# jakub-zarzycki2022/gym-PBN-stac

Measured on AMD Instinct MI355X. Metric: env-steps/sec (whole node), Bittner-200, batch=1M; achieved HBM GB/s, higher is better.
Workload: dtype u64; 1 GPU; Bittner-200 async node update (R1 Graph.step), step mode: one update per env per launch, state resident in device memory; network=bittner199, n_nodes=199, state_words=4, batch_per_gpu=1048576, global_batch=1048576, parallelism=dp1 (env shards, no collective), rng=philox4x32-10

## Files before the change

gym-pbn-stac_amd/csrc/pbn_abi.cpp:

```cpp
#include "pbn_host.hpp"

#include <cstdlib>

const void* DevCache::on(int device, const void* host, size_t bytes) {
    std::lock_guard<std::mutex> g(mu);
    auto it = dev.find(device);
    if (it != dev.end()) return it->second;
    void* p = nullptr;
    if (hipMalloc(&p, bytes) != hipSuccess) return nullptr;
    if (hipMemcpy(p, host, bytes, hipMemcpyHostToDevice) != hipSuccess) {
        (void)hipFree(p);
        return nullptr;
    }
    dev[device] = p;
    return p;
}

void DevCache::release() {
    for (auto& kv : dev) {
        (void)hipSetDevice(kv.first);
        (void)hipFree(kv.second);
    }
    dev.clear();
}
// ... 5 lines not shown
    if (const char* v = getenv("PBNSIM_STEP_BLOCK")) k.step_block = atoi(v) == 256 ? 256 : 1024;
    k.env_no_gen = getenv("PBNSIM_ENV_NO_GEN") != nullptr;
    if (const char* v = getenv("PBNSIM_ENV_GROUP")) k.env_group = std::max(1, atoi(v));
    if (const char* v = getenv("PBNSIM_ENV_BPC")) k.env_bpc = std::max(1, atoi(v));
    if (const char* v = getenv("PBNSIM_ENV_CHUNK")) k.env_chunk = atoi(v);
    if (const char* v = getenv("PBNSIM_ENV_GRID")) k.env_grid_cap = std::max(1, atoi(v));
    if (const char* v = getenv("PBNSIM_ENV_TAIL")) k.env_tail = std::max(0, std::min(64, atoi(v)));
    if (const char* v = getenv("PBNSIM_ENV_LANES")) k.env_lane_limit = std::max(0, std::min(64, atoi(v)));
    if (const char* v = getenv("PBNSIM_ENV_STEAL")) k.env_steal = atoi(v) != 0;
    if (const char* v = getenv("PBNSIM_ENV_KERNEL_IMAGE")) k.env_kernel_image = atoi(v) != 0;
    if (const char* v = getenv("PBNSIM_ENV_HELPERS")) k.env_helpers = std::max(0, std::min(3, atoi(v)));
    if (const char* v = getenv("PBNSIM_ENV_GRID_STEAL")) k.env_grid_steal = atoi(v) != 0 ? 1 : 0;
#ifdef PBN_MEASURE_KNOBS
    if (const char* v = getenv("PBNSIM_ENV_POOL_CU_IDLE")) k.env_pool_cu_idle = atoi(v) != 0 ? 1 : 0;
    if (const char* v = getenv("PBNSIM_ENV_GRID_SLOTS")) k.env_grid_slots = std::max(1, std::min((int)GPOOL_CAP, atoi(v)));
#endif
    if (const char* v = getenv("PBNSIM_SSD_WAVE")) k.ssd_wave = atoi(v) ? 1 : 0;
    if (const char* v = getenv("PBNSIM_SSD_SERIAL")) k.ssd_serial = atoi(v) != 0;
    if (const char* v = getenv("PBNSIM_SSD_SHARED")) {
        const int w = atoi(v);
        k.ssd_shared = w == 0 ? 0 : (w == 4 || w == 8) ? w : 1;
    }
    if (const char* v = getenv("PBNSIM_STEP_GRAPH")) k.step_graph = atoi(v) != 0 ? 1 : 0;
    if (const char* v = getenv("PBNSIM_MT_LANES")) k.mt_lane_walk = atoi(v) != 0;
    if (const char* v = getenv("PBNSIM_ROLL_GROUP")) k.roll_group = std::max(0, atoi(v));
    return k;
}

static bool roll_group_ok(const pbn_net* net) { return net->kind == PBN_KIND_PREDICTOR_MIX && net->N <= 256; }

static int roll_group_size(const pbn_batch* b, const pbn_net* net) {
    if (!roll_group_ok(net)) return 1;
    const uint64_t lanes = (uint64_t)b->n_cu * 512u;
    for (int g = 8; g >= 2; g /= 2)
        if (b->B * (uint64_t)g <= lanes) return g;
    return 1;
}

static int check_state_words(const pbn_batch* b, const uint64_t* w) {
    const int r = b->N & 63;
    if (!r) return 0;
    const uint64_t bad = ~(((uint64_t)1 << r) - 1);
    for (uint64_t e = 0; e < b->B; e++)
        if (w[e * b->W + b->W - 1] & bad) return fail(PBN_E_RANGE, "env %llu has bits set beyond node %d",
                                                       (unsigned long long)e, b->N - 1);
    return 0;
}

int h2d(pbn_batch* b, void* dst, const void* src, size_t bytes) {
    if (bytes <= PinBuf::CAP && b->pin.ready()) {
        HIP_TRY(hipStreamSynchronize(b->stream));
        memcpy(b->pin.p, src, bytes);
        HIP_TRY(hipMemcpyAsync(dst, b->pin.p, bytes, hipMemcpyHostToDevice, b->stream));
    } else {
        HIP_TRY(hipMemcpyAsync(dst, src, bytes, hipMemcpyHostToDevice, b->stream));
    }
    return 0;
}

// ... 106 lines not shown
    if (n_envs < 1) return fail(PBN_E_INVALID, "n_envs must be >= 1");
    if (env_id_base + n_envs > ((uint64_t)1 << 56)) return fail(PBN_E_RANGE, "global env ids must stay below 2^56");
    if (int rc = open_device(device)) return rc;
    pbn_batch* b = new pbn_batch;
    b->net = net;
    b->device = device;
    b->W = net->W;
    b->N = net->N;
    b->B = n_envs;
    b->env_base = env_id_base;
    b->seed = seed;
    b->knob = read_knobs();
    hipDeviceProp_t prop;
    int rc = 0;
    auto bail = [&](int code) {
        pbn_batch_destroy(b);
        return code;
    };
    if (hipGetDeviceProperties(&prop, device) != hipSuccess) return bail(fail(PBN_E_HIP, "hipGetDeviceProperties"));
    b->n_cu = prop.multiProcessorCount;
    if (b->knob.step_block)
        b->step_block = b->knob.step_block;
    else
        b->step_block = n_envs >= (uint64_t)b->n_cu * 1024u * (uint64_t)b->knob.envs_per_thread ? 1024 : 256;
    b->sg.off = b->knob.step_graph >= 0 ? b->knob.step_graph == 0 : n_envs * (uint64_t)b->W >= STEP_GRAPH_MAX_WORDS;
    b->roll_group = roll_group_size(b, net);
    if (b->knob.roll_group >= 0) {
        const int g = b->knob.roll_group;
        b->roll_group = (g == 2 || g == 4 || g == 8) && roll_group_ok(net) ? g : 1;
    }
    if (hipStreamCreateWithFlags(&b->stream, hipStreamNonBlocking) != hipSuccess)
        return bail(fail(PBN_E_HIP, "hipStreamCreate"));
    b->own_stream = b->stream;
    size_t sb = 8 * (size_t)b->W * n_envs;
    if (hipMalloc(&b->d_state, sb) != hipSuccess) return bail(fail(PBN_E_NOMEM, "state alloc (%zu B)", sb));
    if (hipMalloc(&b->d_nsteps, 8 * n_envs) != hipSuccess) return bail(fail(PBN_E_NOMEM, "n_steps alloc"));
    if (hipMalloc(&b->d_error, 8) != hipSuccess) return bail(fail(PBN_E_NOMEM, "error flag alloc"));
    if (hipMemsetAsync(b->d_error, 0, 8, b->stream) != hipSuccess || hipMemsetAsync(b->d_state, 0, sb, b->stream) != hipSuccess ||
        hipMemsetAsync(b->d_nsteps, 0, 8 * n_envs, b->stream) != hipSuccess)
        return bail(fail(PBN_E_HIP, "hipMemset"));
    b->d_image = net->image_on(device);
    if (!b->d_image) return bail(fail(PBN_E_NOMEM, "network image upload failed"));
    if ((rc = max_blocks_step(b->W, net->kind, net->L.bytes, BLOCK, &b->bpc_base)))
        return bail(fail(PBN_E_HIP, "occupancy query: %s", hipGetErrorString((hipError_t)rc)));
    if ((rc = max_blocks_step(b->W, net->kind, net->L.plane_off, b->step_block, &b->bpc_step)))
        return bail(fail(PBN_E_HIP, "occupancy query: %s", hipGetErrorString((hipError_t)rc)));
    if ((rc = max_blocks_step(b->W, net->kind, net->L.plane_off, BLOCK, &b->bpc_roll, 1, b->roll_group)))
        return bail(fail(PBN_E_HIP, "occupancy query: %s", hipGetErrorString((hipError_t)rc)));
    if (hipStreamSynchronize(b->stream) != hipSuccess) return bail(fail(PBN_E_HIP, "stream sync"));
    *out = b;
    return 0;
}
void pbn_batch_destroy(pbn_batch* b) {
    if (!b) return;
    (void)hipSetDevice(b->device);
    if (b->stream) (void)hipStreamSynchronize(b->stream);
    for (auto& pr : b->tm.ev_pool) {
        (void)hipEventDestroy(pr.first);
        (void)hipEventDestroy(pr.second);
    }
    if (b->d_state) (void)hipFree(b->d_state);
    if (b->d_nsteps) (void)hipFree(b->d_nsteps);
    if (b->d_error) (void)hipFree(b->d_error);
    for (DevBuf* d : {&b->s_act, &b->s_obs, &b->s_rew, &b->s_flags, &b->s_nup, &b->s_replay_i, &b->s_replay_k,
                      &b->s_off, &b->s_mask, &b->mt.py, &b->mt.np, &b->mt.pos_py, &b->mt.pos_np, &b->mt.seeds,
                      &b->r6.counter, &b->r6.steal, &b->r6.gpool, &b->aux.ssd_hist, &b->aux.ssd_tab, &b->aux.sync_tab, &b->sg.ubase, &b->s_flip_err})
        d->release();
    for (hipGraphExec_t& g : b->sg.graph)
        if (g) (void)hipGraphExecDestroy(g);
    for (hipGraphExec_t& g : b->sg.exact_graph)
        if (g) (void)hipGraphExecDestroy(g);
    b->pin.release();
    if (b->own_stream) {
        (void)hipStreamSynchronize(b->stream);
        (void)hipStreamDestroy(b->own_stream);
    }
    delete b;
}

int pbn_batch_set_stream(pbn_batch* b, int own, void* stream) {
    CHECK_NN(b, "batch");
    hipStream_t s = own ? b->own_stream : (hipStream_t)stream;
    if (s == b->stream) return 0;
    SET_DEV(b);
    HIP_TRY(hipStreamSynchronize(b->stream));
    b->stream = s;
    return 0;
}

int pbn_batch_get_info(const pbn_batch* b, pbn_batch_info* info) {
    CHECK_NN(b, "batch");
    CHECK_NN(info, "info");
    info->n_nodes = b->N;
    info->n_words = b->W;
    info->kind = b->net->kind;
    info->device = b->device;
    info->n_envs = b->B;
    info->env_id_base = b->env_base;
    info->seed = b->seed;
    info->update_count = b->update_count;
    info->env_call_count = b->r6.calls;
    info->reset_count = b->reset_count;
    info->mt_ready = b->mt.ready;
    const EnvPlan& p = b->r6.last;
    info->env_lanes = p.grp;
    info->roll_lanes = b->roll_group;
    info->env_grid = p.grid;
    info->env_kernel = p.kernel;
    info->env_lane_limit = (int)p.lane_limit;
    info->env_handoff = p.handoff ? 1 : 0;
    info->env_chunk = (p.mode == ENV_MODE_COOP || p.mode == ENV_MODE_TAIL) ? (int)p.chunk : 0;
    return 0;
}

int pbn_sync(pbn_batch* b) {
    CHECK_NN(b, "batch");
    SET_DEV(b);
    HIP_TRY(hipStreamSynchronize(b->stream));
    if (b->r6.fault_check) {
        b->r6.fault_check = false;
        int32_t f = 0;
        HIP_TRY(hipMemcpy(&f, b->d_error + 1, 4, hipMemcpyDeviceToHost));
        if (f) {
            HIP_TRY(hipMemset(b->d_error + 1, 0, 4));
            return fail(PBN_E_HIP, "k_env grid pool: a wait timed out in a device-path launch (an env's outputs "
                                   "were not written)");
        }
    }
    return 0;
}

int pbn_set_state(pbn_batch* b, const uint64_t* words) {
    CHECK_NN(b, "batch");
    CHECK_NN(words, "words");
// ... 190 lines not shown
```

gym-pbn-stac_amd/csrc/pbn_abi_sim.cpp:

```cpp
#include "pbn_host.hpp"

static int step_launch(pbn_batch* b, uint32_t T, uint64_t update_base, int replay, const void* d_i, const void* d_k,
                       const uint64_t* ubase_dev = nullptr, bool timed = true) {
    StepArgs a{};
    a.ubase_dev = ubase_dev;
    a.state = b->d_state;
    a.img = b->d_image;
    a.L = b->net->L;
    a.B = b->B;
    a.env_base = b->env_base;
    a.seed = b->seed;
    a.update_base = update_base;
    a.T = T;
    a.replay_node = (const uint32_t*)d_i;
    a.replay_k53 = (const uint64_t*)d_k;
    hipEvent_t stop = nullptr;
    if (timed)
        if (int rc = b->ev_begin(&stop)) return rc;
    int store = (T == 1 && !replay) ? b->knob.store_mode : STORE_FULL;
    const bool rollout = T > 1 && !replay;
    a.grp = rollout ? b->roll_group : 1;
    const uint64_t K = rollout ? 1u : (uint64_t)b->knob.envs_per_thread;
    const uint64_t lanes = rollout ? b->B * (uint64_t)a.grp : (b->B + K - 1) / K;
    const int sb = (replay || rollout) ? BLOCK : b->step_block;
    const int grid = replay    ? b->grid_for(lanes, b->bpc_base)
                     : rollout ? b->grid_for(lanes, b->bpc_roll, sb)
                               : b->grid_for(lanes, b->bpc_step, sb);
    int e = launch_step(b->W, a, store, replay, sb, grid, b->stream);
    if (e) return fail(PBN_E_HIP, "k_step launch: %s", hipGetErrorString((hipError_t)e));
    return timed ? b->ev_end(stop) : 0;
}

static bool step_graph_ready(pbn_batch* b) {
    if (b->sg.built) return true;
    if (b->sg.broken || b->sg.off || !b->stream) return false;
    if (b->sg.ubase.ensure(64)) return false;
    bool ok = true;
    for (int j = 0; ok && j < STEP_GRAPH_SIZES; ++j) {
        const uint32_t K = STEP_GRAPH_K >> j;
        hipGraph_t g = nullptr;
        ok = hipStreamBeginCapture(b->stream, hipStreamCaptureModeThreadLocal) == hipSuccess;
        bool launched = ok;
        for (uint32_t k = 0; launched && k < K; ++k)
            launched = step_launch(b, 1, k, 0, nullptr, nullptr, (const uint64_t*)b->sg.ubase.p, false) == 0;
        if (launched) launched = launch_bump((uint64_t*)b->sg.ubase.p, K, b->stream) == 0;
        if (ok) ok = hipStreamEndCapture(b->stream, &g) == hipSuccess && launched && g;
        if (ok) ok = hipGraphInstantiate(&b->sg.graph[j], g, nullptr, nullptr, 0) == hipSuccess;
        if (g) (void)hipGraphDestroy(g);
    }
    if (!ok) {
        for (hipGraphExec_t& g : b->sg.graph) {
            if (g) (void)hipGraphExecDestroy(g);
            g = nullptr;
        }
        b->sg.broken = true;
        (void)hipGetLastError();
        g_err.clear();
        return false;
    }
    b->sg.built = true;
    return true;
}

static int exact_graph_build(pbn_batch* b, uint32_t n) {
    if (n < 2 || n > STEP_GRAPH_K || b->sg.broken || b->sg.off || b->sg.exact_broken || !b->stream)
        return -1;
    if (b->sg.ubase.ensure(64)) return -1;
    hipGraph_t g = nullptr;
    hipGraphExec_t x = nullptr;
    bool ok = hipStreamBeginCapture(b->stream, hipStreamCaptureModeThreadLocal) == hipSuccess;
    bool launched = ok;
    for (uint32_t k = 0; launched && k < n; ++k)
        launched = step_launch(b, 1, k, 0, nullptr, nullptr, (const uint64_t*)b->sg.ubase.p, false) == 0;
    if (ok) ok = hipStreamEndCapture(b->stream, &g) == hipSuccess && launched && g;
    if (ok) ok = hipGraphInstantiate(&x, g, nullptr, nullptr, 0) == hipSuccess;
    if (ok) ok = hipGraphUpload(x, b->stream) == hipSuccess;
    if (g) (void)hipGraphDestroy(g);
    if (!ok) {
        if (x) (void)hipGraphExecDestroy(x);
        b->sg.exact_broken = true;
        (void)hipGetLastError();
        g_err.clear();
        return -1;
    }
    int slot = 0;
    for (int j = 1; j < pbn_batch::StepGraphs::EXACT_GRAPHS; ++j)
        if (b->sg.exact_used[j] < b->sg.exact_used[slot]) slot = j;
    if (b->sg.exact_graph[slot]) {
        if (hipStreamSynchronize(b->stream) != hipSuccess) {
            (void)hipGraphExecDestroy(x);
            (void)fail(PBN_E_HIP, "stream sync before graph eviction failed");
            return -1;
        }
        (void)hipGraphExecDestroy(b->sg.exact_graph[slot]);
    }
    b->sg.exact_graph[slot] = x;
    b->sg.exact_n[slot] = n;
    b->sg.exact_used[slot] = ++b->sg.exact_clock;
    return slot;
}

static int exact_graph_find(pbn_batch* b, uint32_t n) {
    for (int j = 0; j < pbn_batch::StepGraphs::EXACT_GRAPHS; ++j)
        if (b->sg.exact_graph[j] && b->sg.exact_n[j] == n) return j;
    return -1;
}

static bool stream_capturing(pbn_batch* b) {
    hipStreamCaptureStatus cap = hipStreamCaptureStatusNone;
    if (b->stream && hipStreamIsCapturing(b->stream, &cap) != hipSuccess) return true;
    return cap != hipStreamCaptureStatusNone;
}

static int upload_update_count(pbn_batch* b) {
    uint32_t* c = (uint32_t*)b->sg.ubase.p;
    HIP_TRY(hipMemsetD32Async((hipDeviceptr_t)c, (int)(uint32_t)b->update_count, 1, b->stream));
    HIP_TRY(hipMemsetD32Async((hipDeviceptr_t)(c + 1), (int)(uint32_t)(b->update_count >> 32), 1, b->stream));
    return 0;
}

static int check_replay_nodes(const pbn_batch* b, const char* what, const uint32_t* node_idx, const uint64_t* k53,
                              uint64_t n) {
    const uint32_t lo = (uint32_t)b->net->kind == PBN_KIND_PROB_TABLE ? 1u : 0u;
    for (uint64_t q = 0; q < n; q++) {
        if (node_idx[q] >= (uint32_t)b->N || node_idx[q] < lo)
            return fail(PBN_E_RANGE, "%s node index %u outside [%u, %d)", what, node_idx[q], lo, b->N);
        if (k53 && k53[q] >> 53) return fail(PBN_E_RANGE, "replay k53 must be < 2^53");
    }
    return 0;
}

extern "C" {

int pbn_step_prepare(pbn_batch* b, uint32_t n_updates) {
    CHECK_NN(b, "batch");
    if (n_updates > PBN_STEP_PREPARE_MAX)
        return fail(PBN_E_INVALID, "n_updates=%u above PBN_STEP_PREPARE_MAX", n_updates);
    SET_DEV(b);
    if (n_updates < 2 || b->sg.off || stream_capturing(b)) return 0;
    if (n_updates > STEP_GRAPH_K) (void)step_graph_ready(b);
    else if (exact_graph_find(b, n_updates) < 0) (void)exact_graph_build(b, n_updates);
    return 0;
}

int pbn_step(pbn_batch* b, uint32_t n_updates) {
    CHECK_NN(b, "batch");
    SET_DEV(b);
    uint32_t t = 0;
    const bool cap = stream_capturing(b);
    const uint32_t smallest = STEP_GRAPH_K >> (STEP_GRAPH_SIZES - 1);
    int exact = -1;
    if (!cap && b->tm.mode != 1 && n_updates >= 2 && !b->sg.off) {
        exact = exact_graph_find(b, n_updates);
        if (exact < 0 && n_updates == b->sg.last_n && n_updates <= STEP_GRAPH_K)
            exact = exact_graph_build(b, n_updates);
    }
    b->sg.last_n = n_updates;
    if (exact >= 0) {
        if (int rc = upload_update_count(b)) return rc;
        hipEvent_t stop;
        if (int rc = b->ev_begin(&stop)) return rc;
        if (b->tm.mode == 2) b->tm.region_launches += n_updates - 1;
        HIP_TRY(hipGraphLaunch(b->sg.exact_graph[exact], b->stream));
        if (int rc = b->ev_end(stop)) return rc;
        b->sg.exact_used[exact] = ++b->sg.exact_clock;
        b->update_count += n_updates;
        return 0;
    }
    if (n_updates >= smallest && b->tm.mode != 1 && !cap && step_graph_ready(b)) {
        if (int rc = upload_update_count(b)) return rc;
        for (int j = 0; j < STEP_GRAPH_SIZES; ++j) {
            const uint32_t K = STEP_GRAPH_K >> j;
            while (n_updates - t >= K && (j == 0 || n_updates - t < 2 * K)) {
                hipEvent_t stop;
                if (int rc = b->ev_begin(&stop)) return rc;
                if (b->tm.mode == 2) b->tm.region_launches += K - 1;
                HIP_TRY(hipGraphLaunch(b->sg.graph[j], b->stream));
                if (int rc = b->ev_end(stop)) return rc;
                b->update_count += K;
                t += K;
            }
        }
    }
    for (; t < n_updates; t++) {
        if (int rc = step_launch(b, 1, b->update_count, 0, nullptr, nullptr)) return rc;
        b->update_count++;
    }
    return 0;
}

int pbn_rollout(pbn_batch* b, uint32_t n_updates) {
    CHECK_NN(b, "batch");
    if (!n_updates) return 0;
    SET_DEV(b);
    if (int rc = step_launch(b, n_updates, b->update_count, 0, nullptr, nullptr)) return rc;
    b->update_count += n_updates;
    return 0;
}

int pbn_step_replay(pbn_batch* b, const uint32_t* node_idx, const uint64_t* k53, uint32_t n_updates) {
    CHECK_NN(b, "batch");
    if (!n_updates) return 0;
    CHECK_NN(node_idx, "node_idx");
    CHECK_NN(k53, "k53");
    const uint64_t n = (uint64_t)n_updates * b->B;
    if (int rc = check_replay_nodes(b, "replay", node_idx, k53, n)) return rc;
    SET_DEV(b);
    if (int rc = b->s_replay_i.ensure(4 * n)) return rc;
    if (int rc = b->s_replay_k.ensure(8 * n)) return rc;
    HIP_TRY(hipMemcpyAsync(b->s_replay_i.p, node_idx, 4 * n, hipMemcpyHostToDevice, b->stream));
    HIP_TRY(hipMemcpyAsync(b->s_replay_k.p, k53, 8 * n, hipMemcpyHostToDevice, b->stream));
    if (int rc = step_launch(b, n_updates, 0, 1, b->s_replay_i.p, b->s_replay_k.p)) return rc;
    HIP_TRY(hipStreamSynchronize(b->stream));
    return 0;
}

int pbn_step_forced(pbn_batch* b, const uint32_t* node_idx, uint32_t n_updates) {
    CHECK_NN(b, "batch");
    if (!n_updates) return 0;
    CHECK_NN(node_idx, "node_idx");
    const uint64_t n = (uint64_t)n_updates * b->B;
    if (int rc = check_replay_nodes(b, "forced", node_idx, nullptr, n)) return rc;
    SET_DEV(b);
    if (int rc = b->s_replay_i.ensure(4 * n)) return rc;
    HIP_TRY(hipMemcpyAsync(b->s_replay_i.p, node_idx, 4 * n, hipMemcpyHostToDevice, b->stream));
    if (int rc = step_launch(b, n_updates, b->update_count, 1, b->s_replay_i.p, nullptr)) return rc;
    b->update_count += n_updates;
    HIP_TRY(hipStreamSynchronize(b->stream));
    return 0;
}

static MTArgs mt_args(pbn_batch* b) {
    MTArgs a{};
    a.state = b->d_state;
    a.img = b->d_image;
    a.L = b->net->L;
    a.B = b->B;
    a.n_nodes = b->N;
    a.mt_py = (uint32_t*)b->mt.py.p;
    a.mt_np = (uint32_t*)b->mt.np.p;
    a.pos_py = (uint32_t*)b->mt.pos_py.p;
    a.pos_np = (uint32_t*)b->mt.pos_np.p;
    a.lane_walk = b->knob.mt_lane_walk ? 1 : 0;
    return a;
}

int pbn_mt_seed(pbn_batch* b, const uint64_t* seeds, int init_state) {
    CHECK_NN(b, "batch");
    CHECK_NN(seeds, "seeds");
// ... 135 lines not shown
```

gym-pbn-stac_amd/csrc/pbn_host.hpp:

```cpp
#pragma once
#include <algorithm>
#include <cstdint>
#include <cstring>
#include <map>
#include <mutex>
#include <string>
#include <vector>

#ifndef PBN_HOST_NO_HIP
#include <hip/hip_runtime_api.h>
#endif

#include "../../include/pbn_abi.h"
#include "pbn_params.hpp"

using namespace pbn;

#define PBN_HIDDEN __attribute__((visibility("hidden")))

extern PBN_HIDDEN thread_local std::string g_err;
PBN_HIDDEN int fail(int code, const char* fmt, ...) __attribute__((format(printf, 2, 3)));

#define CHECK_NN(p, name) \
    if (!(p)) return fail(PBN_E_INVALID, "%s is NULL", name)

inline uint32_t align16(uint32_t x) { return (x + 15u) & ~15u; }

struct DevCache {
    std::mutex mu;
    std::map<int, void*> dev;
    PBN_HIDDEN const void* on(int device, const void* host, size_t bytes);
    PBN_HIDDEN void release();
};

struct pbn_net {
    int kind = 0, N = 0, W = 0;
// ... 63 lines not shown
    }
};

inline int open_device(int device) {
    int ndev = 0;
    hipError_t e = hipGetDeviceCount(&ndev);
    if (e != hipSuccess || ndev < 1)
        return fail(PBN_E_HIP, "no HIP device available (hipGetDeviceCount: %s); libpbnsim has no CPU path",
                    hipGetErrorString(e));
    if (device < 0 || device >= ndev) return fail(PBN_E_RANGE, "device %d outside [0, %d)", device, ndev);
    HIP_TRY(hipSetDevice(device));
    return 0;
}

inline int check_action_shape(int A, int offset) {
    if (A < 1 || A > 4096) return fail(PBN_E_INVALID, "A=%d outside [1, 4096]", A);
    if (offset != 0 && offset != 1) return fail(PBN_E_INVALID, "offset must be 0 or 1");
    return 0;
}

constexpr uint32_t STEP_GRAPH_K = 64;
constexpr int STEP_GRAPH_SIZES = 6;
constexpr uint64_t STEP_GRAPH_MAX_WORDS = 1ull << 20;

struct Knobs {
    int store_mode = STORE_DIRTY;
    int envs_per_thread = 2;
    int step_block = 0;
    int step_graph = -1;
    int roll_group = -1;
    bool env_no_gen = false;
    int env_group = 0;
    int env_bpc = 0;
    int env_chunk = 0;
    int env_grid_cap = 0;
    int env_tail = -1;
    int env_lane_limit = 0;
    bool env_steal = true;
    bool env_kernel_image = false;
    int env_helpers = 3;
    int env_grid_steal = -1;
    int env_pool_cu_idle = -1;
    int env_grid_slots = 0;
    int ssd_wave = -1;
    bool ssd_serial = false;
    int ssd_shared = -1;
    bool mt_lane_walk = false;
};

struct EnvPlan {
    int mode = -1;
    int grp = 0;
// ... 10 lines not shown
};

struct pbn_batch {
    pbn_net* net = nullptr;
    int device = 0, W = 0, N = 0;
    hipStream_t stream = nullptr;
    hipStream_t own_stream = nullptr;
    uint64_t B = 0, env_base = 0, seed = 0, update_count = 0;
    uint32_t reset_count = 0;
    uint64_t* d_state = nullptr;
    int64_t* d_nsteps = nullptr;
    int32_t* d_error = nullptr;
    const void* d_image = nullptr;
    int n_cu = 0, bpc_step = 1, bpc_base = 1, bpc_roll = 1;
    int step_block = 1024;
    int roll_group = 1;
    Knobs knob;
    PinBuf pin;
    DevBuf s_flip_err;
    DevBuf s_act, s_obs, s_rew, s_flags, s_nup, s_replay_i, s_replay_k, s_off, s_mask;

    struct StepGraphs {
        bool off = false;
        hipGraphExec_t graph[STEP_GRAPH_SIZES] = {};
        bool built = false;
        bool broken = false;
        bool exact_broken = false;
        static constexpr int EXACT_GRAPHS = 4;
        uint32_t exact_n[EXACT_GRAPHS] = {};
        hipGraphExec_t exact_graph[EXACT_GRAPHS] = {};
        uint64_t exact_used[EXACT_GRAPHS] = {};
        uint64_t exact_clock = 0;
        uint32_t last_n = 0;
        DevBuf ubase;
    } sg;
    struct R6 {
        uint32_t calls = 0;
        DevBuf counter;
        DevBuf steal;
        DevBuf gpool;
        uint32_t gpool_epoch = 0;
        bool fault_check = false;
        EnvPlan last;
    } r6;
    struct MT {
        DevBuf py, np, pos_py, pos_np, seeds;
        int ready = 0;
    } mt;
    struct Aux {
        DevBuf ssd_hist, ssd_tab;
        uint64_t ssd_iters = 0;
        DevBuf sync_tab;
        uint64_t sync_steps = 0;
    } aux;
    struct Timing {
        int mode = 0;
        std::vector<std::pair<hipEvent_t, hipEvent_t>> ev_pool;
        size_t ev_used = 0;
// ... 118 lines not shown
```

gym-pbn-stac_amd/csrc/pbn_params.hpp:

```cpp
#pragma once
#include <stdint.h>

namespace pbn {

enum { KIND_PREDICTOR_MIX = 1, KIND_PROB_TABLE = 2 };
enum {
    STREAM_STEP = 1,
    STREAM_INIT = 2,
    STREAM_ENV = 3,
    STREAM_RESET = 4,
    STREAM_SSD = 5,
    STREAM_SSD_FLIP = 6,
    STREAM_SYNC = 7,
    STREAM_SYNC_PERT = 8
};
enum { STORE_FULL = 0, STORE_DIRTY = 1 };
enum EnvMode {
    ENV_MODE_CUBES = 0,
    ENV_MODE_COUNTERS = 1,
    ENV_MODE_COOP = 2,
    ENV_MODE_GROUP = 3,
    ENV_MODE_TAIL = 4
};

// ... 214 lines not shown
struct ReachArgs {
    const void* img;
    NetLayout L;
    uint64_t* keys;
    uint32_t* mark;
    unsigned long long* table;
    uint32_t* ctl;
    uint32_t* queue;
    uint32_t* free_ring;
    unsigned long long* hull;
    const uint64_t* in;
    uint64_t* out;
    uint64_t n_in;
    uint32_t tmask, key_cap, max_states, fmask;
    uint32_t free_limit;
    uint32_t free_any;
    uint32_t lo, hi;
    uint32_t epoch;
};

enum { REACH_K_UNSTABLE = 0, REACH_K_SEED, REACH_K_EXPAND, REACH_K_BACK_START, REACH_K_BACK, REACH_K_HULL };
int launch_reach(int W, int which, const ReachArgs& a, int grid, void* stream);
int launch_bump(uint64_t* p, uint64_t k, void* stream);
int launch_step(int W, const StepArgs& a, int store_mode, int replay, int sb, int grid, void* stream);
uint32_t step_lds_bytes(int W, uint32_t image_bytes, int sb, int grp = 1);
int launch_init(int W, const InitArgs& a, int grid, void* stream);
int launch_flip(int W, const FlipArgs& a, int grid, void* stream);
int launch_unpack(const uint64_t* words, uint8_t* out, uint64_t B, uint32_t N, uint32_t W, int grid, void* stream);
int launch_env_multi(int W, const EnvArgs& a, int replay, int grid, void* stream);
int max_blocks_step(int W, int kind, uint32_t lds_bytes, int sb, int* blocks_per_cu, int rollout = 0, int grp = 1);

#ifndef PBN_ENV_CHUNK
#define PBN_ENV_CHUNK 32
#endif
constexpr uint32_t ENV_CHUNK = PBN_ENV_CHUNK;
#ifndef PBN_ENV_UNROLL
#define PBN_ENV_UNROLL 8
#endif
constexpr uint32_t ENV_UNROLL = PBN_ENV_UNROLL;
constexpr uint32_t ENV_TAIL_DEFAULT = 16;
constexpr uint64_t ENV_ONE_LANE_ENVS_PER_SLOT = 6;
constexpr uint32_t ENV_CHUNK_SMALL = 32, ENV_CHUNK_LARGE = 48;
constexpr uint32_t env_gen_wave_bytes(uint32_t chunk) { return chunk * 64u * 2u + 64u + 64u * 16u; }
int max_blocks_env(int W, int kind, int fast, int grp, uint32_t lds_bytes, int* blocks_per_cu, uint32_t chunk = ENV_CHUNK_LARGE);
uint32_t env_lds_bytes(int W, uint32_t image_bytes, int fast, int grp, uint32_t chunk = ENV_CHUNK_LARGE);
inline int env_block(int fast) { return fast == ENV_MODE_GROUP ? BLOCK : ENV_BLOCK; }
// ... 10 lines not shown
```

gym-pbn-stac_amd/csrc/pbn_step.hip:

```cpp
#include <hip/hip_runtime.h>

#include "pbn_device.hpp"
#include "pbn_launch.hpp"
#include "pbn_params.hpp"

namespace pbn {

#ifdef PBN_STAMPS
__device__ uint64_t g_stamps[16384 * 8];
#endif

template <int W, int KIND, int STORE, int SB, bool PRE = false>
__device__ __forceinline__ void k_step_single(const StepArgs& a, uint8_t* lds, uint64_t e, uint64_t stride,
                                              uint64_t (&cur)[W], uint32_t N, uint64_t (*pre_nxt)[W] = nullptr) {
    const uint64_t u = a.update_base + (a.ubase_dev ? *a.ubase_dev : 0ull);
    const uint64_t po = stride;
    uint64_t nxt[W];
    uint32_t i0 = 0, i1 = 0;
    uint64_t q0 = 0, q1 = 0;
    const bool paired = (a.env_base & 1u) == 0u;
    const bool odd = (threadIdx.x & 1u) != 0u;
    auto draws = [&](uint64_t ea) {
        const uint64_t g0 = a.env_base + ea, g1 = g0 + po;
        uint32_t n0, c0, n1, c1;
// ... 379 lines not shown
    return (int)hipMemcpyToSymbol(HIP_SYMBOL(g_stamps), z, sizeof z, 0, hipMemcpyHostToDevice);
}
}
extern "C" int pbn_exp_stamps(void* out, size_t bytes) {
    return (int)hipMemcpyFromSymbol(out, HIP_SYMBOL(pbn::g_stamps), bytes, 0, hipMemcpyDeviceToHost);
}
extern "C" int pbn_exp_stamps_clear() {
    int rc = pbn::step_stamps_clear();
    if (!rc) rc = pbn::env_stamps_clear();
    return rc;
}
namespace pbn {
#endif

__global__ void k_bump(uint64_t* p, uint64_t k) {
    if (threadIdx.x == 0) p[threadIdx.x] += k;
}

int launch_bump(uint64_t* p, uint64_t k, void* stream) {
    void* kargs[] = {(void*)&p, (void*)&k};
    return (int)hipLaunchKernel((const void*)k_bump, dim3(1), dim3(64), kargs, 0, (hipStream_t)stream);
}

}
```

gym-pbn-stac_amd/gym_pbn_amd/_lib.py:

```python

from __future__ import annotations

import ctypes as C
import os
from pathlib import Path

try:
    import torch
except Exception:
    torch = None

PKG_DIR = Path(__file__).resolve().parent
LIB_PATH = Path(os.environ.get("PBNSIM_LIB", PKG_DIR / "libpbnsim.so"))

PBN_OK = 0
PBN_E_INVALID = -1
PBN_E_RANGE = -2
PBN_E_HIP = -3
PBN_E_NOMEM = -4
PBN_E_UNSUPPORTED = -5
PBN_E_STATE = -6

FLAG_TERMINATED = 1
FLAG_TRUNCATED = 2
# ... 9 lines not shown


class PbnError(RuntimeError):
    def __init__(self, code: int, msg: str):
        super().__init__(f"[{code}] {msg}")
        self.code = code


class NetDesc(C.Structure):
    _fields_ = [
        ("kind", C.c_int32), ("n_nodes", C.c_int32), ("n_preds", C.c_int32),
        ("pred_offsets", _i32p), ("pred_inputs", _i32p), ("pred_tt", _u16p), ("pred_thr", _u64p),
        ("node_k", _i32p), ("input_offsets", _i32p), ("inputs", _i32p), ("thr_offsets", _i64p), ("thr", _u64p),
    ]


class BatchInfo(C.Structure):
    _fields_ = [
        ("n_nodes", C.c_int32), ("n_words", C.c_int32), ("kind", C.c_int32), ("device", C.c_int32),
        ("n_envs", C.c_uint64), ("env_id_base", C.c_uint64), ("seed", C.c_uint64), ("update_count", C.c_uint64),
        ("env_call_count", C.c_uint32), ("reset_count", C.c_uint32), ("mt_ready", C.c_int32),
        ("env_lanes", C.c_int32), ("roll_lanes", C.c_int32), ("env_grid", C.c_int32), ("env_kernel", C.c_int32),
        ("env_lane_limit", C.c_int32), ("env_handoff", C.c_int32), ("env_chunk", C.c_int32),
    ]


class EnvCfgDesc(C.Structure):
    _fields_ = [
        ("n_cubes", C.c_int32), ("cube_care", _u64p), ("cube_value", _u64p),
        ("n_reset_cubes", C.c_int32), ("reset_care", _u64p), ("reset_value", _u64p),
        ("target_care", _u64p), ("target_value", _u64p),
        ("horizon", C.c_int32), ("reward_success", C.c_int32), ("action_cost", C.c_int32),
        ("first_update_tested", C.c_int32),
    ]


class ReachInfo(C.Structure):
    _fields_ = [
        ("n_nodes", C.c_int32), ("n_words", C.c_int32), ("device", C.c_int32), ("complete", C.c_int32),
        ("max_states", C.c_uint64), ("table_slots", C.c_uint64), ("key_capacity", C.c_uint64),
        ("n_states", C.c_uint64), ("n_entries", C.c_uint64),
    ]


_PP = C.POINTER(_vp)

# ... 101 lines not shown
```

include/pbn_abi.h:

```cpp
#ifndef PBN_ABI_H
#define PBN_ABI_H

#include <stdint.h>

#ifdef __cplusplus
extern "C" {
#endif

#define PBN_ABI_VERSION 15

enum {
    PBN_OK = 0,
    PBN_E_INVALID = -1,
    PBN_E_RANGE = -2,
    PBN_E_HIP = -3,
    PBN_E_NOMEM = -4,
    PBN_E_UNSUPPORTED = -5,
    PBN_E_STATE = -6
};

enum { PBN_KIND_PREDICTOR_MIX = 1, PBN_KIND_PROB_TABLE = 2 };

typedef struct pbn_net pbn_net;
typedef struct pbn_batch pbn_batch;
typedef struct pbn_envcfg pbn_envcfg;
typedef struct pbn_reach pbn_reach;

typedef struct {
    int32_t kind;
    int32_t n_nodes;
    int32_t n_preds;
    const int32_t *pred_offsets;
    const int32_t *pred_inputs;
    const uint16_t *pred_tt;
    const uint64_t *pred_thr;
    const int32_t *node_k;
    const int32_t *input_offsets;
    const int32_t *inputs;
    const int64_t *thr_offsets;
    const uint64_t *thr;
} pbn_net_desc;

typedef struct {
    int32_t n_nodes, n_words, kind, device;
    uint64_t n_envs, env_id_base, seed;
    uint64_t update_count;
    uint32_t env_call_count, reset_count;
    int32_t mt_ready;
    int32_t env_lanes;
    int32_t roll_lanes;
    int32_t env_grid;
    int32_t env_kernel;
    int32_t env_lane_limit;
    int32_t env_handoff;
    int32_t env_chunk;
} pbn_batch_info;

typedef struct {
    int32_t n_cubes;
    const uint64_t *cube_care;
    const uint64_t *cube_value;
    int32_t n_reset_cubes;
    const uint64_t *reset_care;
    const uint64_t *reset_value;
    const uint64_t *target_care;
    const uint64_t *target_value;
    int32_t horizon;
    int32_t reward_success;
    int32_t action_cost;
    int32_t first_update_tested;
} pbn_envcfg_desc;

enum { PBN_FLAG_TERMINATED = 1, PBN_FLAG_TRUNCATED = 2, PBN_FLAG_CAPPED = 4 };

int pbn_abi_version(void);
const char *pbn_last_error(void);
int pbn_device_count(int *count);

// ... 86 lines not shown
```

Before: 163.2 billion env-steps/s.

## Split step batch into parallel stream chains with per-chain graphs

Splits the env batch into up to four contiguous slices and runs each slice's sequence of step kernels on its own stream, joined to the main stream through fork and join events. Per-chain hipGraphs, with their own update counters, are captured for both the power-of-two and the exact-n paths, and graph capture is now allowed for larger batches when chains are used. The aim is to overlap kernel tails and launch gaps between consecutive one-update launches across independent slices. In exchange it adds stream and event overhead, needs more graph memory, and each slice keeps fewer resident lanes.

```diff
diff --git a/gym-pbn-stac_amd/csrc/pbn_abi.cpp b/gym-pbn-stac_amd/csrc/pbn_abi.cpp
--- a/gym-pbn-stac_amd/csrc/pbn_abi.cpp
+++ b/gym-pbn-stac_amd/csrc/pbn_abi.cpp
@@ -51,6 +51,10 @@
         k.ssd_shared = w == 0 ? 0 : (w == 4 || w == 8) ? w : 1;
     }
     if (const char* v = getenv("PBNSIM_STEP_GRAPH")) k.step_graph = atoi(v) != 0 ? 1 : 0;
+    if (const char* v = getenv("PBNSIM_STEP_CHAINS")) {
+        const int s = atoi(v);
+        k.step_chains = s >= 4 ? 4 : s >= 2 ? 2 : 1;
+    }
     if (const char* v = getenv("PBNSIM_MT_LANES")) k.mt_lane_walk = atoi(v) != 0;
     if (const char* v = getenv("PBNSIM_ROLL_GROUP")) k.roll_group = std::max(0, atoi(v));
     return k;
@@ -64,6 +68,15 @@
     for (int g = 8; g >= 2; g /= 2)
         if (b->B * (uint64_t)g <= lanes) return g;
     return 1;
+}
+
+static uint64_t step_fill_envs(const pbn_batch* b) {
+    return (uint64_t)b->n_cu * 1024u * (uint64_t)b->knob.envs_per_thread;
+}
+
+static int step_chains_for(const pbn_batch* b) {
+    if (b->knob.step_chains) return b->knob.step_chains;
+    return b->step_block == 1024 && b->B >= 2 * step_fill_envs(b) ? 2 : 1;
 }
 
 static int check_state_words(const pbn_batch* b, const uint64_t* w) {
@@ -216,8 +229,12 @@
     if (b->knob.step_block)
         b->step_block = b->knob.step_block;
     else
-        b->step_block = n_envs >= (uint64_t)b->n_cu * 1024u * (uint64_t)b->knob.envs_per_thread ? 1024 : 256;
-    b->sg.off = b->knob.step_graph >= 0 ? b->knob.step_graph == 0 : n_envs * (uint64_t)b->W >= STEP_GRAPH_MAX_WORDS;
+        b->step_block = n_envs >= step_fill_envs(b) ? 1024 : 256;
+    b->ch.n = chain_split(n_envs, step_chains_for(b), b->step_block, b->ch.sl);
+    b->ch.min_updates = b->knob.step_chains ? 2u : STEP_CHAIN_MIN_UPDATES;
+    b->sg.off = b->knob.step_graph >= 0 ? b->knob.step_graph == 0
+                                        : n_envs * (uint64_t)b->W >=
+                                              (b->ch.n > 1 ? STEP_CHAIN_GRAPH_MAX_WORDS : STEP_GRAPH_MAX_WORDS);
     b->roll_group = roll_group_size(b, net);
     if (b->knob.roll_group >= 0) {
         const int g = b->knob.roll_group;
@@ -226,6 +243,14 @@
     if (hipStreamCreateWithFlags(&b->stream, hipStreamNonBlocking) != hipSuccess)
         return bail(fail(PBN_E_HIP, "hipStreamCreate"));
     b->own_stream = b->stream;
+    if (b->ch.n > 1) {
+        for (int c = 1; c < b->ch.n; ++c)
+            if (hipStreamCreateWithFlags(&b->ch.stream[c], hipStreamNonBlocking) != hipSuccess ||
+                hipEventCreateWithFlags(&b->ch.done[c], hipEventDisableTiming) != hipSuccess)
+                return bail(fail(PBN_E_HIP, "step chain %d: stream / event create", c));
+        if (hipEventCreateWithFlags(&b->ch.fork, hipEventDisableTiming) != hipSuccess)
+            return bail(fail(PBN_E_HIP, "step chains: event create"));
+    }
     size_t sb = 8 * (size_t)b->W * n_envs;
     if (hipMalloc(&b->d_state, sb) != hipSuccess) return bail(fail(PBN_E_NOMEM, "state alloc (%zu B)", sb));
     if (hipMalloc(&b->d_nsteps, 8 * n_envs) != hipSuccess) return bail(fail(PBN_E_NOMEM, "n_steps alloc"));
@@ -249,6 +274,14 @@
     if (!b) return;
     (void)hipSetDevice(b->device);
     if (b->stream) (void)hipStreamSynchronize(b->stream);
+    for (int c = 1; c < STEP_CHAINS_MAX; ++c) {
+        if (b->ch.stream[c]) {
+            (void)hipStreamSynchronize(b->ch.stream[c]);
+            (void)hipStreamDestroy(b->ch.stream[c]);
+        }
+        if (b->ch.done[c]) (void)hipEventDestroy(b->ch.done[c]);
+    }
+    if (b->ch.fork) (void)hipEventDestroy(b->ch.fork);
     for (auto& pr : b->tm.ev_pool) {
         (void)hipEventDestroy(pr.first);
         (void)hipEventDestroy(pr.second);
@@ -260,10 +293,12 @@
                       &b->s_off, &b->s_mask, &b->mt.py, &b->mt.np, &b->mt.pos_py, &b->mt.pos_np, &b->mt.seeds,
                       &b->r6.counter, &b->r6.steal, &b->r6.gpool, &b->aux.ssd_hist, &b->aux.ssd_tab, &b->aux.sync_tab, &b->sg.ubase, &b->s_flip_err})
         d->release();
-    for (hipGraphExec_t& g : b->sg.graph)
-        if (g) (void)hipGraphExecDestroy(g);
-    for (hipGraphExec_t& g : b->sg.exact_graph)
-        if (g) (void)hipGraphExecDestroy(g);
+    for (auto& chain : b->sg.graph)
+        for (hipGraphExec_t& g : chain)
+            if (g) (void)hipGraphExecDestroy(g);
+    for (auto& slot : b->sg.exact_graph)
+        for (hipGraphExec_t& g : slot)
+            if (g) (void)hipGraphExecDestroy(g);
     b->pin.release();
     if (b->own_stream) {
         (void)hipStreamSynchronize(b->stream);
@@ -304,6 +339,7 @@
     info->env_lane_limit = (int)p.lane_limit;
     info->env_handoff = p.handoff ? 1 : 0;
     info->env_chunk = (p.mode == ENV_MODE_COOP || p.mode == ENV_MODE_TAIL) ? (int)p.chunk : 0;
+    info->step_chains = b->ch.n;
     return 0;
 }
 
diff --git a/gym-pbn-stac_amd/csrc/pbn_abi_sim.cpp b/gym-pbn-stac_amd/csrc/pbn_abi_sim.cpp
--- a/gym-pbn-stac_amd/csrc/pbn_abi_sim.cpp
+++ b/gym-pbn-stac_amd/csrc/pbn_abi_sim.cpp
@@ -1,14 +1,23 @@
 #include "pbn_host.hpp"
 
-static int step_launch(pbn_batch* b, uint32_t T, uint64_t update_base, int replay, const void* d_i, const void* d_k,
-                       const uint64_t* ubase_dev = nullptr, bool timed = true) {
+struct StepRange {
+    uint64_t off, len;
+    hipStream_t stream;
+};
+static StepRange whole_batch(const pbn_batch* b) { return {0, b->B, b->stream}; }
+static StepRange chain_range(const pbn_batch* b, int c, hipStream_t stream) {
+    return {b->ch.sl[c].off, b->ch.sl[c].len, stream};
+}
+
+static int step_launch(pbn_batch* b, const StepRange& r, uint32_t T, uint64_t update_base, int replay, const void* d_i,
+                       const void* d_k, const uint64_t* ubase_dev = nullptr, bool timed = true) {
     StepArgs a{};
     a.ubase_dev = ubase_dev;
-    a.state = b->d_state;
+    a.state = b->d_state + r.off * (uint64_t)b->W;
     a.img = b->d_image;
     a.L = b->net->L;
-    a.B = b->B;
-    a.env_base = b->env_base;
+    a.B = r.len;
+    a.env_base = b->env_base + r.off;
     a.seed = b->seed;
     a.update_base = update_base;
     a.T = T;
@@ -21,12 +30,12 @@
     const bool rollout = T > 1 && !replay;
     a.grp = rollout ? b->roll_group : 1;
     const uint64_t K = rollout ? 1u : (uint64_t)b->knob.envs_per_thread;
-    const uint64_t lanes = rollout ? b->B * (uint64_t)a.grp : (b->B + K - 1) / K;
+    const uint64_t lanes = rollout ? r.len * (uint64_t)a.grp : (r.len + K - 1) / K;
     const int sb = (replay || rollout) ? BLOCK : b->step_block;
     const int grid = replay    ? b->grid_for(lanes, b->bpc_base)
                      : rollout ? b->grid_for(lanes, b->bpc_roll, sb)
                                : b->grid_for(lanes, b->bpc_step, sb);
-    int e = launch_step(b->W, a, store, replay, sb, grid, b->stream);
+    int e = launch_step(b->W, a, store, replay, sb, grid, r.stream);
     if (e) return fail(PBN_E_HIP, "k_step launch: %s", hipGetErrorString((hipError_t)e));
     return timed ? b->ev_end(stop) : 0;
 }
@@ -36,23 +45,27 @@
     if (b->sg.broken || b->sg.off || !b->stream) return false;
     if (b->sg.ubase.ensure(64)) return false;
     bool ok = true;
-    for (int j = 0; ok && j < STEP_GRAPH_SIZES; ++j) {
-        const uint32_t K = STEP_GRAPH_K >> j;
-        hipGraph_t g = nullptr;
-        ok = hipStreamBeginCapture(b->stream, hipStreamCaptureModeThreadLocal) == hipSuccess;
-        bool launched = ok;
-        for (uint32_t k = 0; launched && k < K; ++k)
-            launched = step_launch(b, 1, k, 0, nullptr, nullptr, (const uint64_t*)b->sg.ubase.p, false) == 0;
-        if (launched) launched = launch_bump((uint64_t*)b->sg.ubase.p, K, b->stream) == 0;
-        if (ok) ok = hipStreamEndCapture(b->stream, &g) == hipSuccess && launched && g;
-        if (ok) ok = hipGraphInstantiate(&b->sg.graph[j], g, nullptr, nullptr, 0) == hipSuccess;
-        if (g) (void)hipGraphDestroy(g);
-    }
+    for (int c = 0; ok && c < b->ch.n; ++c)
+        for (int j = 0; ok && j < STEP_GRAPH_SIZES; ++j) {
+            const uint32_t K = STEP_GRAPH_K >> j;
+            uint64_t* counter = (uint64_t*)b->sg.ubase.p + c;
+            const StepRange r = chain_range(b, c, b->stream);
+            hipGraph_t g = nullptr;
+            ok = hipStreamBeginCapture(b->stream, hipStreamCaptureModeThreadLocal) == hipSuccess;
+            bool launched = ok;
+            for (uint32_t k = 0; launched && k < K; ++k)
+                launched = step_launch(b, r, 1, k, 0, nullptr, nullptr, counter, false) == 0;
+            if (launched) launched = launch_bump(counter, K, b->stream) == 0;
+            if (ok) ok = hipStreamEndCapture(b->stream, &g) == hipSuccess && launched && g;
+            if (ok) ok = hipGraphInstantiate(&b->sg.graph[c][j], g, nullptr, nullptr, 0) == hipSuccess;
+            if (g) (void)hipGraphDestroy(g);
+        }
     if (!ok) {
-        for (hipGraphExec_t& g : b->sg.graph) {
-            if (g) (void)hipGraphExecDestroy(g);
-            g = nullptr;
-        }
+        for (auto& chain : b->sg.graph)
+            for (hipGraphExec_t& g : chain) {
+                if (g) (void)hipGraphExecDestroy(g);
+                g = nullptr;
+            }
         b->sg.broken = true;
         (void)hipGetLastError();
         g_err.clear();
@@ -66,18 +79,27 @@
     if (n < 2 || n > STEP_GRAPH_K || b->sg.broken || b->sg.off || b->sg.exact_broken || !b->stream)
         return -1;
     if (b->sg.ubase.ensure(64)) return -1;
-    hipGraph_t g = nullptr;
-    hipGraphExec_t x = nullptr;
-    bool ok = hipStreamBeginCapture(b->stream, hipStreamCaptureModeThreadLocal) == hipSuccess;
-    bool launched = ok;
-    for (uint32_t k = 0; launched && k < n; ++k)
-        launched = step_launch(b, 1, k, 0, nullptr, nullptr, (const uint64_t*)b->sg.ubase.p, false) == 0;
-    if (ok) ok = hipStreamEndCapture(b->stream, &g) == hipSuccess && launched && g;
-    if (ok) ok = hipGraphInstantiate(&x, g, nullptr, nullptr, 0) == hipSuccess;
-    if (ok) ok = hipGraphUpload(x, b->stream) == hipSuccess;
-    if (g) (void)hipGraphDestroy(g);
+    hipGraphExec_t x[STEP_CHAINS_MAX] = {};
+    bool ok = true;
+    for (int c = 0; ok && c < b->ch.n; ++c) {
+        const StepRange r = chain_range(b, c, b->stream);
+        hipGraph_t g = nullptr;
+        ok = hipStreamBeginCapture(b->stream, hipStreamCaptureModeThreadLocal) == hipSuccess;
+        bool launched = ok;
+        for (uint32_t k = 0; launched && k < n; ++k)
+            launched = step_launch(b, r, 1, k, 0, nullptr, nullptr, (const uint64_t*)b->sg.ubase.p + c, false) == 0;
+        if (ok) ok = hipStreamEndCapture(b->stream, &g) == hipSuccess && launched && g;
+        if (ok) ok = hipGraphInstantiate(&x[c], g, nullptr, nullptr, 0) == hipSuccess;
+        if (ok) ok = hipGraphUpload(x[c], b->chain_stream(c)) == hipSuccess;
+        if (g) (void)hipGraphDestroy(g);
+    }
+    for (int c = 1; c < b->ch.n; ++c) (void)hipStreamSynchronize(b->ch.stream[c]);
+    auto drop = [&] {
+        for (hipGraphExec_t& e : x)
+            if (e) (void)hipGraphExecDestroy(e);
+    };
     if (!ok) {
-        if (x) (void)hipGraphExecDestroy(x);
+        drop();
         b->sg.exact_broken = true;
         (void)hipGetLastError();
         g_err.clear();
@@ -86,15 +108,16 @@
     int slot = 0;
     for (int j = 1; j < pbn_batch::StepGraphs::EXACT_GRAPHS; ++j)
         if (b->sg.exact_used[j] < b->sg.exact_used[slot]) slot = j;
-    if (b->sg.exact_graph[slot]) {
+    if (b->sg.exact_graph[slot][0]) {
         if (hipStreamSynchronize(b->stream) != hipSuccess) {
-            (void)hipGraphExecDestroy(x);
+            drop();
             (void)fail(PBN_E_HIP, "stream sync before graph eviction failed");
             return -1;
         }
-        (void)hipGraphExecDestroy(b->sg.exact_graph[slot]);
-    }
-    b->sg.exact_graph[slot] = x;
+        for (hipGraphExec_t& e : b->sg.exact_graph[slot])
+            if (e) (void)hipGraphExecDestroy(e);
+    }
+    for (int c = 0; c < STEP_CHAINS_MAX; ++c) b->sg.exact_graph[slot][c] = x[c];
     b->sg.exact_n[slot] = n;
     b->sg.exact_used[slot] = ++b->sg.exact_clock;
     return slot;
@@ -102,7 +125,7 @@
 
 static int exact_graph_find(pbn_batch* b, uint32_t n) {
     for (int j = 0; j < pbn_batch::StepGraphs::EXACT_GRAPHS; ++j)
-        if (b->sg.exact_graph[j] && b->sg.exact_n[j] == n) return j;
+        if (b->sg.exact_graph[j][0] && b->sg.exact_n[j] == n) return j;
     return -1;
 }
 
@@ -113,9 +136,22 @@
 }
 
 static int upload_update_count(pbn_batch* b) {
-    uint32_t* c = (uint32_t*)b->sg.ubase.p;
-    HIP_TRY(hipMemsetD32Async((hipDeviceptr_t)c, (int)(uint32_t)b->update_count, 1, b->stream));
-    HIP_TRY(hipMemsetD32Async((hipDeviceptr_t)(c + 1), (int)(uint32_t)(b->update_count >> 32), 1, b->stream));
+    if (int e = launch_set_counters((uint64_t*)b->sg.ubase.p, b->update_count, (uint32_t)b->ch.n, b->stream))
+        return fail(PBN_E_HIP, "k_set_counters launch: %s", hipGetErrorString((hipError_t)e));
+    return 0;
+}
+
+static int chains_fork(pbn_batch* b) {
+    HIP_TRY(hipEventRecord(b->ch.fork, b->stream));
+    for (int c = 1; c < b->ch.n; ++c) HIP_TRY(hipStreamWaitEvent(b->ch.stream[c], b->ch.fork, 0));
+    return 0;
+}
+
+static int chains_join(pbn_batch* b) {
+    for (int c = 1; c < b->ch.n; ++c) {
+        HIP_TRY(hipEventRecord(b->ch.done[c], b->ch.stream[c]));
+        HIP_TRY(hipStreamWaitEvent(b->stream, b->ch.done[c], 0));
+    }
     return 0;
 }
 
@@ -138,6 +174,7 @@
         return fail(PBN_E_INVALID, "n_updates=%u above PBN_STEP_PREPARE_MAX", n_updates);
     SET_DEV(b);
     if (n_updates < 2 || b->sg.off || stream_capturing(b)) return 0;
+    if (b->ch.n > 1 && n_updates < b->ch.min_updates) return 0;
     if (n_updates > STEP_GRAPH_K) (void)step_graph_ready(b);
     else if (exact_graph_find(b, n_updates) < 0) (void)exact_graph_build(b, n_updates);
     return 0;
@@ -149,51 +186,80 @@
     uint32_t t = 0;
     const bool cap = stream_capturing(b);
     const uint32_t smallest = STEP_GRAPH_K >> (STEP_GRAPH_SIZES - 1);
+    const bool run = !cap && b->tm.mode != 1 && n_updates >= 2;
+    const bool chained = run && b->ch.n > 1 && n_updates >= b->ch.min_updates;
+    const int S = chained ? b->ch.n : 1;
+    const bool graphs = run && !b->sg.off && (b->ch.n == 1 || chained);
     int exact = -1;
-    if (!cap && b->tm.mode != 1 && n_updates >= 2 && !b->sg.off) {
+    if (graphs) {
         exact = exact_graph_find(b, n_updates);
         if (exact < 0 && n_updates == b->sg.last_n && n_updates <= STEP_GRAPH_K)
             exact = exact_graph_build(b, n_updates);
     }
     b->sg.last_n = n_updates;
-    if (exact >= 0) {
+    const bool pow2 = exact < 0 && graphs && n_updates >= smallest && step_graph_ready(b);
+    if (exact >= 0 || pow2)
         if (int rc = upload_update_count(b)) return rc;
+    if (chained) {
+        if (b->tm.mode == 2) {
+            hipEvent_t stop;
+            if (int rc = b->ev_begin(&stop)) return rc;
+            b->tm.region_launches += n_updates - 1;
+        }
+        if (int rc = chains_fork(b)) return rc;
+    }
+    auto count = [&](uint32_t k) -> int {
+        if (chained) return 0;
         hipEvent_t stop;
         if (int rc = b->ev_begin(&stop)) return rc;
-        if (b->tm.mode == 2) b->tm.region_launches += n_updates - 1;
-        HIP_TRY(hipGraphLaunch(b->sg.exact_graph[exact], b->stream));
-        if (int rc = b->ev_end(stop)) return rc;
-        b->sg.exact_used[exact] = ++b->sg.exact_clock;
-        b->update_count += n_updates;
+        if (b->tm.mode == 2) b->tm.region_launches += k - 1;
         return 0;
-    }
-    if (n_updates >= smallest && b->tm.mode != 1 && !cap && step_graph_ready(b)) {
-        if (int rc = upload_update_count(b)) return rc;
-        for (int j = 0; j < STEP_GRAPH_SIZES; ++j) {
-            const uint32_t K = STEP_GRAPH_K >> j;
-            while (n_updates - t >= K && (j == 0 || n_updates - t < 2 * K)) {
-                hipEvent_t stop;
-                if (int rc = b->ev_begin(&stop)) return rc;
-                if (b->tm.mode == 2) b->tm.region_launches += K - 1;
-                HIP_TRY(hipGraphLaunch(b->sg.graph[j], b->stream));
-                if (int rc = b->ev_end(stop)) return rc;
-                b->update_count += K;
-                t += K;
+    };
+    auto queue = [&]() -> int {
+        if (exact >= 0) {
+            if (int rc = count(n_updates)) return rc;
+            for (int c = 0; c < S; ++c) HIP_TRY(hipGraphLaunch(b->sg.exact_graph[exact][c], b->chain_stream(c)));
+            b->sg.exact_used[exact] = ++b->sg.exact_clock;
+            b->update_count += n_updates;
+            return 0;
+        }
+        if (pow2) {
+            for (int j = 0; j < STEP_GRAPH_SIZES; ++j) {
+                const uint32_t K = STEP_GRAPH_K >> j;
+                while (n_updates - t >= K && (j == 0 || n_updates - t < 2 * K)) {
+                    if (int rc = count(K)) return rc;
+                    for (int c = 0; c < S; ++c) HIP_TRY(hipGraphLaunch(b->sg.graph[c][j], b->chain_stream(c)));
+                    b->update_count += K;
+                    t += K;
+                }
             }
         }
-    }
-    for (; t < n_updates; t++) {
-        if (int rc = step_launch(b, 1, b->update_count, 0, nullptr, nullptr)) return rc;
-        b->update_count++;
-    }
-    return 0;
+        for (; t < n_updates; t++) {
+            if (!chained) {
+                if (int rc = step_launch(b, whole_batch(b), 1, b->update_count, 0, nullptr, nullptr)) return rc;
+            } else {
+                for (int c = 0; c < S; ++c)
+                    if (int rc = step_launch(b, chain_range(b, c, b->chain_stream(c)), 1, b->update_count, 0, nullptr,
+                                             nullptr, nullptr, false))
+                        return rc;
+            }
+            b->update_count++;
+        }
+        return 0;
+    };
+    int rc = queue();
+    if (chained) {
+        const int jrc = chains_join(b);
+        if (!rc) rc = jrc;
+    }
+    return rc;
 }
 
 int pbn_rollout(pbn_batch* b, uint32_t n_updates) {
     CHECK_NN(b, "batch");
     if (!n_updates) return 0;
     SET_DEV(b);
-    if (int rc = step_launch(b, n_updates, b->update_count, 0, nullptr, nullptr)) return rc;
+    if (int rc = step_launch(b, whole_batch(b), n_updates, b->update_count, 0, nullptr, nullptr)) return rc;
     b->update_count += n_updates;
     return 0;
 }
@@ -210,7 +276,7 @@
     if (int rc = b->s_replay_k.ensure(8 * n)) return rc;
     HIP_TRY(hipMemcpyAsync(b->s_replay_i.p, node_idx, 4 * n, hipMemcpyHostToDevice, b->stream));
     HIP_TRY(hipMemcpyAsync(b->s_replay_k.p, k53, 8 * n, hipMemcpyHostToDevice, b->stream));
-    if (int rc = step_launch(b, n_updates, 0, 1, b->s_replay_i.p, b->s_replay_k.p)) return rc;
+    if (int rc = step_launch(b, whole_batch(b), n_updates, 0, 1, b->s_replay_i.p, b->s_replay_k.p)) return rc;
     HIP_TRY(hipStreamSynchronize(b->stream));
     return 0;
 }
@@ -224,7 +290,7 @@
     SET_DEV(b);
     if (int rc = b->s_replay_i.ensure(4 * n)) return rc;
     HIP_TRY(hipMemcpyAsync(b->s_replay_i.p, node_idx, 4 * n, hipMemcpyHostToDevice, b->stream));
-    if (int rc = step_launch(b, n_updates, b->update_count, 1, b->s_replay_i.p, nullptr)) return rc;
+    if (int rc = step_launch(b, whole_batch(b), n_updates, b->update_count, 1, b->s_replay_i.p, nullptr)) return rc;
     b->update_count += n_updates;
     HIP_TRY(hipStreamSynchronize(b->stream));
     return 0;
diff --git a/gym-pbn-stac_amd/csrc/pbn_chain_split.hpp b/gym-pbn-stac_amd/csrc/pbn_chain_split.hpp
--- /dev/null
+++ b/gym-pbn-stac_amd/csrc/pbn_chain_split.hpp
@@ -0,0 +1,31 @@
+#pragma once
+#include <cstdint>
+
+namespace pbn {
+
+constexpr int STEP_CHAINS_MAX = 4;
+
+struct ChainSlice {
+    uint64_t off = 0, len = 0;
+};
+
+inline int chain_split(uint64_t B, int S, int step_block, ChainSlice (&out)[STEP_CHAINS_MAX]) {
+    if (S > STEP_CHAINS_MAX) S = STEP_CHAINS_MAX;
+    if (S < 1) S = 1;
+    const uint64_t big = 2ull * (uint64_t)(step_block > 0 ? step_block : 1);
+    const uint64_t unit = B >= (uint64_t)S * big ? big : 2ull;
+    const uint64_t units = (B + unit - 1) / unit;
+    if (units < (uint64_t)S) S = units ? (int)units : 1;
+    const uint64_t per = units / (uint64_t)S, extra = units % (uint64_t)S;
+    uint64_t at = 0;
+    for (int c = 0; c < S; ++c) {
+        const uint64_t end = at + (per + ((uint64_t)c < extra ? 1u : 0u)) * unit;
+        out[c].off = at;
+        out[c].len = (end < B ? end : B) - at;
+        at = end < B ? end : B;
+    }
+    for (int c = S; c < STEP_CHAINS_MAX; ++c) out[c] = ChainSlice{};
+    return S;
+}
+
+}
diff --git a/gym-pbn-stac_amd/csrc/pbn_host.hpp b/gym-pbn-stac_amd/csrc/pbn_host.hpp
--- a/gym-pbn-stac_amd/csrc/pbn_host.hpp
+++ b/gym-pbn-stac_amd/csrc/pbn_host.hpp
@@ -12,6 +12,7 @@
 #endif
 
 #include "../../include/pbn_abi.h"
+#include "pbn_chain_split.hpp"
 #include "pbn_params.hpp"
 
 using namespace pbn;
@@ -121,12 +122,15 @@
 constexpr uint32_t STEP_GRAPH_K = 64;
 constexpr int STEP_GRAPH_SIZES = 6;
 constexpr uint64_t STEP_GRAPH_MAX_WORDS = 1ull << 20;
+constexpr uint64_t STEP_CHAIN_GRAPH_MAX_WORDS = 1ull << 24;
+constexpr uint32_t STEP_CHAIN_MIN_UPDATES = 128;
 
 struct Knobs {
     int store_mode = STORE_DIRTY;
     int envs_per_thread = 2;
     int step_block = 0;
     int step_graph = -1;
+    int step_chains = 0;
     int roll_group = -1;
     bool env_no_gen = false;
     int env_group = 0;
@@ -183,18 +187,27 @@
 
     struct StepGraphs {
         bool off = false;
-        hipGraphExec_t graph[STEP_GRAPH_SIZES] = {};
+        hipGraphExec_t graph[STEP_CHAINS_MAX][STEP_GRAPH_SIZES] = {};
         bool built = false;
         bool broken = false;
         bool exact_broken = false;
         static constexpr int EXACT_GRAPHS = 4;
         uint32_t exact_n[EXACT_GRAPHS] = {};
-        hipGraphExec_t exact_graph[EXACT_GRAPHS] = {};
+        hipGraphExec_t exact_graph[EXACT_GRAPHS][STEP_CHAINS_MAX] = {};
         uint64_t exact_used[EXACT_GRAPHS] = {};
         uint64_t exact_clock = 0;
         uint32_t last_n = 0;
         DevBuf ubase;
     } sg;
+    struct Chains {
+        int n = 1;
+        uint32_t min_updates = 2;
+        ChainSlice sl[STEP_CHAINS_MAX];
+        hipStream_t stream[STEP_CHAINS_MAX] = {};
+        hipEvent_t done[STEP_CHAINS_MAX] = {};
+        hipEvent_t fork = nullptr;
+    } ch;
+    hipStream_t chain_stream(int c) const { return c ? ch.stream[c] : stream; }
     struct R6 {
         uint32_t calls = 0;
         DevBuf counter;
diff --git a/gym-pbn-stac_amd/csrc/pbn_params.hpp b/gym-pbn-stac_amd/csrc/pbn_params.hpp
--- a/gym-pbn-stac_amd/csrc/pbn_params.hpp
+++ b/gym-pbn-stac_amd/csrc/pbn_params.hpp
@@ -260,6 +260,7 @@
 enum { REACH_K_UNSTABLE = 0, REACH_K_SEED, REACH_K_EXPAND, REACH_K_BACK_START, REACH_K_BACK, REACH_K_HULL };
 int launch_reach(int W, int which, const ReachArgs& a, int grid, void* stream);
 int launch_bump(uint64_t* p, uint64_t k, void* stream);
+int launch_set_counters(uint64_t* p, uint64_t v, uint32_t n, void* stream);
 int launch_step(int W, const StepArgs& a, int store_mode, int replay, int sb, int grid, void* stream);
 uint32_t step_lds_bytes(int W, uint32_t image_bytes, int sb, int grp = 1);
 int launch_init(int W, const InitArgs& a, int grid, void* stream);
diff --git a/gym-pbn-stac_amd/csrc/pbn_step.hip b/gym-pbn-stac_amd/csrc/pbn_step.hip
--- a/gym-pbn-stac_amd/csrc/pbn_step.hip
+++ b/gym-pbn-stac_amd/csrc/pbn_step.hip
@@ -425,4 +425,14 @@
     return (int)hipLaunchKernel((const void*)k_bump, dim3(1), dim3(64), kargs, 0, (hipStream_t)stream);
 }
 
-}
+__global__ void k_set_counters(uint64_t* p, uint64_t v, uint32_t n) {
+    if (threadIdx.x < n) p[threadIdx.x] = v;
+}
+
+int launch_set_counters(uint64_t* p, uint64_t v, uint32_t n, void* stream) {
+    if (n > 64u) return (int)hipErrorInvalidValue;
+    void* kargs[] = {(void*)&p, (void*)&v, (void*)&n};
+    return (int)hipLaunchKernel((const void*)k_set_counters, dim3(1), dim3(64), kargs, 0, (hipStream_t)stream);
+}
+
+}
diff --git a/gym-pbn-stac_amd/gym_pbn_amd/_lib.py b/gym-pbn-stac_amd/gym_pbn_amd/_lib.py
--- a/gym-pbn-stac_amd/gym_pbn_amd/_lib.py
+++ b/gym-pbn-stac_amd/gym_pbn_amd/_lib.py
@@ -55,6 +55,7 @@
         ("env_call_count", C.c_uint32), ("reset_count", C.c_uint32), ("mt_ready", C.c_int32),
         ("env_lanes", C.c_int32), ("roll_lanes", C.c_int32), ("env_grid", C.c_int32), ("env_kernel", C.c_int32),
         ("env_lane_limit", C.c_int32), ("env_handoff", C.c_int32), ("env_chunk", C.c_int32),
+        ("step_chains", C.c_int32),
     ]
 
 
diff --git a/include/pbn_abi.h b/include/pbn_abi.h
--- a/include/pbn_abi.h
+++ b/include/pbn_abi.h
@@ -7,7 +7,7 @@
 extern "C" {
 #endif
 
-#define PBN_ABI_VERSION 15
+#define PBN_ABI_VERSION 16
 
 enum {
     PBN_OK = 0,
@@ -54,6 +54,7 @@
     int32_t env_lane_limit;
     int32_t env_handoff;
     int32_t env_chunk;
+    int32_t step_chains;
 } pbn_batch_info;
 
 typedef struct {
```

Result: faster. 180.8 billion env-steps/s, median of 6 (+10.7%).
